# FrancisGregoryNg/Gaussian_Process_Optimization

Hardware: AMD Instinct MI355X
Metric: GP fit+predict iters/sec at N=16384 D=8 (higher is better)
Workload: dtype f64; 1 GPU; C3 (BASELINE.json configs[2]): N=16384, D=8 RBF iso, fit (K, Cholesky, alpha, LML) + predict mean/var at M=10000 candidates + EI arg-best; candidates_total=10000, candidates_this_rank=10000, entry_point=gp_fit_predict, kernel=RBF, fit=replicated on every rank (does not shard, SURVEY.md 8e), torch_imported=False, launcher=single process, emulate_fp64=0

## Files before the change

### gaussian_process_optimization_amd/csrc/api_core.hip

```cpp
#include "api_internal.h"

thread_local std::string g_err;

static thread_local bool g_note_set = false;
static thread_local std::string g_note_msg;

int fail(int code, const char *fmt, ...) {
    char buf[512];
    va_list ap;
    va_start(ap, fmt);
    vsnprintf(buf, sizeof buf, fmt, ap);
    va_end(ap);
    g_err = buf;
    if (g_note_set) {
        g_err += " [after: " + g_note_msg + "]";
        g_note_set = false;
    }
    return code;
}

void gp_note_hip(hipError_t e, const char *what, const char *file, int line) {
    if (e == hipSuccess || g_note_set) return;
    char buf[512];
    snprintf(buf, sizeof buf, "%s -> %s (%s:%d)", what, hipGetErrorString(e), file, line);
// ... 310 lines not shown
    {"panel_tiles", &gp_ctx::panel_tiles, OPT_RANGE, 1, 64},
    {"inner_tiles", &gp_ctx::inner_tiles, OPT_RANGE, 1, 2},
    {"inner_min_rows", &gp_ctx::inner_min_rows, OPT_FLOOR, 0},
    {"own_keep_per_row", &gp_ctx::own_keep_per_row, OPT_FLOOR, 0},
    {"own_keep_pipe_pct", &gp_ctx::own_keep_pipe_pct, OPT_RANGE, 0, 400},
    {"own_keep_base", &gp_ctx::own_keep_base, OPT_FLOOR, 0},
    {"lookahead", &gp_ctx::lookahead, OPT_BOOL},
    {"lookahead_min_tiles", &gp_ctx::lookahead_min_tiles, OPT_FLOOR, 0},
    {"pipe_start_pct", &gp_ctx::pipe_start_pct, OPT_RANGE, -1, 100},
    {"small_below", &gp_ctx::small_below, OPT_RAW},
    {"pipe_stages_grad", &gp_ctx::pipe_stages_grad, OPT_FLOOR, 0},
    {"pipe_start_pct_grad", &gp_ctx::pipe_start_pct_grad, OPT_RANGE, 0, 100},
    {"pipe_stages", &gp_ctx::pipe_stages, OPT_FLOOR, 0},
    {"lauum_panels", &gp_ctx::lauum_panels, OPT_RAW},
    {"side_alpha", &gp_ctx::side_alpha, OPT_RAW},
    {"pair_panels", &gp_ctx::pair_panels, OPT_BOOL},
    {"pair_tri", &gp_ctx::pair_tri, OPT_RAW},
    {"fmin_direct", &gp_ctx::fmin_direct, OPT_RAW},
    {"chain_small_below", &gp_ctx::chain_small_below, OPT_RAW},
    {"waves8", &gp_ctx::waves8, OPT_BOOL},
    {"stagger", &gp_ctx::stagger, OPT_RAW},
    {"trsm_rows64", &gp_ctx::trsm_rows64, OPT_RAW},
    {"rns_group_fit", &gp_ctx::rns_group_fit, OPT_RANGE, 1, 16},
    {"rns_group", &gp_ctx::rns_group, OPT_RANGE, 1, 16},
    {"emulate_fit", &gp_ctx::emulate_fit, OPT_BOOL},
    {"emulate_fp64", &gp_ctx::emulate_fp64, OPT_BOOL},
    {"rows_build", &gp_ctx::rows_build, OPT_RANGE, -1, 1},
    {"rows_nt", &gp_ctx::rows_nt, OPT_RANGE, -1, 1},
};

// ... 246 lines not shown
```

### gaussian_process_optimization_amd/csrc/api_factor.hip

```cpp
#include "api_internal.h"

void build_ky(gp_ctx *g, const Members &m, bool jittered) {
    launch_kbuild(g->s, m.A, m.lda, g->dX, g->N, g->Npad, m.kp[0], m.diag[0], 0, m.nb, m.sA, m.kpt, m.diag_tab);
    if (jittered) launch_add_diag(g->s, m.A, m.lda, g->N, m.jit[0], m.nb, m.sA, m.jit_tab);
    launch_set_rhs(g->s, m.A, m.lda, g->dY, g->N, g->Npad, g->P, m.nb, m.sA);
}

static int chain_step(gp_ctx *g, hipStream_t s, const Members &m, int j, int J1, int R1) {
    double *A = m.A, *invL = m.invL;
    const long lda = m.lda;
    if (g->inner_tiles >= 2 && m.nb == 1 && j + 1 < J1 && R1 - (j + 2) >= g->inner_min_rows) {
        launch_potrf_pair(s, A, lda, j, invL, m.info);
        launch_trsm2(s, A, lda, j, invL, j + 2, R1);
        if (j + 2 < J1)
            gemm(g, s, 1, A, lda, A + (long)j * GP_TILE, lda, A + (long)j * GP_TILE, lda, 1, 2 * GP_TILE,
                 TileSet{0, R1, j + 2, J1, 1});
        return j + 2;
    }
    launch_potrf_tile(s, A, lda, j, invL, m.info, m.nb, m.sA, m.sI, 4);
    gemm(g, s, 0, A, lda, A + (long)j * GP_TILE, lda, invL + (long)j * GP_TILE * GP_TILE, GP_TILE, 0, GP_TILE,
         TileSet{j + 1, R1, j, j + 1, 0}, member_opt(m, inplace_opt(), m.sA, m.sA, m.sI));
    if (j + 1 < J1)
        gemm(g, s, 1, A, lda, A + (long)j * GP_TILE, lda, A + (long)j * GP_TILE, lda, 1, GP_TILE, TileSet{0, R1, j + 1, J1, 1},
             member_opt(m, GemmOpt(), m.sA, m.sA, m.sA));
// ... 144 lines not shown
            mid_next = 0;
            if (p.edge(J + 3 + Gf) < p.nt) {
                GP_NOTE(hipStreamWaitEvent(sfar, la_event(g, EV_CONV, J), 0));
                rlaunch(sfar, Jg, J1, p.edge(J + 3 + Gf), p.nt, first);
                GP_NOTE(hipEventRecord(la_event(g, EV_FAR, gi), sfar));
                far_issued[gi] = true;
            }
        }
        if (mid_Jg >= 0 && mid_next < Gf) {
            rlaunch(sb, mid_Jg, mid_end, p.edge(mid_base + mid_next), p.edge(mid_base + mid_next + 1), mid_first);
            ++mid_next;
        }
    }
};

int factor_lookahead(gp_ctx *g, const PredPipe &pp) {
    int rc;
    if ((rc = ensure_bulk_stream(g))) return rc;
    const LaPlan p = la_plan(g, pp);
    const int nt = p.nt;
    hipStream_t sp = g->s_panel, sb = g->s_bulk;
    hipStream_t spred = pp.on ? g->s_pred : nullptr, sfar = p.Gf > 1 ? g->s_pred : nullptr;
    if ((rc = reserve_panel_inv(g, p.W, nt))) return rc;
    Members cm = ctx_members(g);
    cm.W = p.W;
    record_wait(g, EV_MISC, 0, g->s, {sp, sb, g->s_inv, spred, sfar});
    if (pp.on && pp.init) pp.init(spred);
    EmuTrail emu{g, p, cm};
    if (p.emu && (rc = emu.prepare())) return rc;
    int next_pred = 0;
    int own_prev = nt;
    for (int J = 0; J < p.nJ; ++J) {
        const int J0 = p.pb[J], J1 = p.pb[J + 1], J2 = p.pb[J + 2];
        for (int j = J0; j < J1;) j = chain_step(g, sp, cm, j, J1, p.R1);
        record_wait(g, EV_CHAIN, J, sp, {g->s_inv});
        build_panel_inv_one(g, g->s_inv, J, p.W, nt);
        if (J < p.pstages) GP_NOTE(hipEventRecord(la_event(g, EV_INVP, J), g->s_inv));
        if (pp.on && J >= p.pred_start) release_stages(g, p, pp, cm, J, &next_pred);
        if (J1 >= nt) break;
        const int oc = p.emu ? nt : first_owned_column(nt, J2, p.W, own_prev, g->own_keep_base, g->own_keep_per_row,
                                                       g->own_keep_pipe_pct, pp.on && J >= p.pred_start);
        own_prev = nt - oc;
        if (oc < nt && J >= 1) panel_update(g, sp, cm, J0, J1, TileSet{0, p.R1, oc, nt, 1});
        if (J >= 1) GP_NOTE(hipStreamWaitEvent(sp, la_event(g, EV_BULK, J - 1), 0));
        panel_update(g, sp, cm, J0, J1, TileSet{0, p.R1, J1, J2, 1});
        if (oc < nt && J == 0)
            panel_update(g, sp, cm, J0, J1, TileSet{0, p.R1, oc, nt, 1});
        if (J2 >= nt) continue;
        GP_NOTE(hipStreamWaitEvent(sb, la_event(g, EV_CHAIN, J), 0));
        if (p.emu) emu.update(J);
        else trail_fp64(g, p, cm, J, oc);
    }
    record_wait(g, EV_MISC, 1, sp, {g->s});
    record_wait(g, EV_MISC, 2, sb, {g->s});
    if (sfar) record_wait(g, EV_MISC, 7, sfar, {g->s});
    g->pipe_done = p.pstages;
    if (spred) record_wait(g, EV_MISC, 3, spred, {g->s});
    record_wait(g, EV_MISC, 4, g->s_inv, {g->s});
// ... 104 lines not shown
        pp->phase = "cholesky+potri_stages";
        pp->rest_phase = "potri_solve_rest";
        pp->flops = (double)N * N * N / 3.0;
        pp->stages = g->pipe_stages_grad;
        if (pp->stages <= 0) pp->stages = std::max(1, (nJ * 36 + 50) / 100);
        pp->start_pct = g->pipe_start_pct_grad;
    }
    return 0;
}

static int factor_attempt(gp_ctx *g, const PredPipe &pp, const double *diag_add, const double *jitter) {
    const double N = (double)g->N;
    const int nt = (int)(g->Npad / GP_TILE);
    g->lr_valid = false;
    g->jitter_try = *jitter;
    int ph = phase_begin(g, "kbuild", 0.0, 8.0 * N * g->D + 8.0 * N * N / 2);
    Members m = ctx_members(g);
    m.diag = diag_add;
    m.jit = jitter;
    build_ky(g, m, *jitter != 0.0);
    phase_end(g, ph);
    HIPCHK(hipMemsetAsync(g->dInfo, 0, sizeof(int) * 4, g->s));
    ph = phase_begin(g, pp.on ? pp.phase : "cholesky", pp.on ? pp.flops : N * N * N / 3.0, 0.0);
    const bool la = pp.on || (g->lookahead && nt > g->panel_tiles && (nt > g->lookahead_min_tiles || emu_fit_applies(g)));
    const int rc = la ? factor_lookahead(g, pp) : factor(g);
    if (rc) return rc;
    phase_end(g, ph);
    return 0;
}

static int rest_stages(gp_ctx *g, const PredPipe &pp, bool *side_alpha) {
    if (g->pipe_done >= pp.nJ) return 0;
    const int phr = phase_begin(g, pp.rest_phase, 0.0, 0.0);
    const int rci = ensure_panel_inv(g);
    if (rci) return rci;
    *side_alpha = g->s_inv && g->side_alpha;
    hipEvent_t eI = la_event(g, EV_MISC, 5);
    if (*side_alpha) GP_NOTE(hipEventRecord(eI, g->s));
    solve_rows(g, ctx_members(g), pp.mt, pp.trapezoid, g->pipe_done);
    if (*side_alpha) {
        GP_NOTE(hipStreamWaitEvent(g->s_inv, eI, 0));
        alpha_lml(g, g->s_inv, ctx_members(g));
        GP_NOTE(hipEventRecord(la_event(g, EV_MISC, 6), g->s_inv));
    }
    phase_end(g, phr);
    return 0;
}

int fit_impl(gp_ctx *g, int maxtries, Pipe kind, int include_noise) {
    HIPCHK(hipSetDevice(g->device));
    QuiesceOnError guard{g};
    const long N = g->N, Npad = g->Npad;
    const int P = g->P;
    int rc;
    PredPipe pp;
    if (kind != Pipe::None && (rc = make_pipe(g, kind, &pp))) return rc;
    double diag_add, diag0;
    ky_diag(g->kp, g->noise, &diag_add, &diag0);
    g->nphases = 0;
    g->emu_off_call = false;
    fit_dropped(g);

    double jitter = 0.0;
    int tries = 0;
    for (int info = 0, bad = 0;;) {
        if ((rc = factor_attempt(g, pp, &diag_add, &jitter))) return rc;
        if ((rc = factor_status(g, g->emulate_fp64 && !g->emu_off_call, &info, &bad))) return rc;
// ... 5 lines not shown
            continue;
        }
        if (info == 0) break;
        g->invp_valid = false;
        const int rcl = ladder_step(diag0, maxtries, info, &jitter, &tries);
        if (rcl == GP_ERR_NOT_PD_DIAG) return fail(rcl, "not pd: non-positive diagonal elements");
        if (rcl) {
            g_err = "not positive definite, even with jitter.";
            return rcl;
        }
        g->nphases = 0;
    }
    g->jitter = jitter;

    bool side_alpha = false;
    if (pp.on && (rc = rest_stages(g, pp, &side_alpha))) return rc;
    if (kind == Pipe::Identity) {
        if ((rc = wi_lauum(g))) return rc;
        g->wi_valid = true;
        g->w_in_t2 = true;
    }
    int ph = phase_begin(g, "alpha_lml", 2.0 * (double)N * N * P, 8.0 * (double)N * N / 2);
    if (side_alpha) {
        GP_NOTE(hipStreamWaitEvent(g->s, la_event(g, EV_MISC, 6), 0));
    } else {
        if ((rc = ensure_panel_inv(g))) return rc;
        alpha_lml(g, g->s, ctx_members(g));
    }
    phase_end(g, ph);
    if (kind == Pipe::Candidates) {
        ph = phase_begin(g, "reduce", 0.0, 8.0 * (double)N * g->M);
        launch_predict_reduce(g->s, g->dT2, Npad, g->M, N, g->dA + Npad * Npad, Npad, P, g->kp.variance,
                              include_noise ? g->noise : 0.0, g->dMean, g->dVar);
        phase_end(g, ph);
    }

    std::vector<double> sc(SCAL_DOT.off + P);
    HIPCHK(hipMemcpyAsync(sc.data(), g->dScal, sizeof(double) * sc.size(), hipMemcpyDeviceToHost, g->s));
    GP_SYNC(g->s);
    g->logdet = sc[SCAL_LOGDET.off];
    g->lml = lml_from_scalars(N, P, sc.data());
    g->fitted = true;
    if (kind == Pipe::Candidates) {
        g->predicted = true;
        g->predicted_noise = include_noise ? 1 : 0;
    }
    guard.armed = false;
    return 0;
// ... 41 lines not shown
```

### gaussian_process_optimization_amd/csrc/api_internal.h

```cpp
#pragma once
#include "gphip_internal.h"
#include "../../include/gphip.h"

#include <hip/hip_ext.h>
#include <rccl/rccl.h>

#include <algorithm>
#include <array>
#include <cmath>
#include <cstdarg>
#include <cstdio>
#include <cstdlib>
#include <cstring>
#include <functional>
#include <map>
#include <mutex>
#include <set>
#include <string>
#include <type_traits>
#include <vector>

extern thread_local std::string g_err;
int fail(int code, const char *fmt, ...);

// ... 108 lines not shown
    __attribute__((noinline)) int grow(long n) {
        const hipError_t e = alloc(n);
        if (e == hipSuccess) return 0;
        return std::is_same<T, double>::value ? fail(GP_ERR_HIP, "hipMalloc(%ld doubles) -> %s", n, hipGetErrorString(e))
                                              : fail(GP_ERR_HIP, "hipMalloc(%ld bytes) -> %s", n * (long)sizeof(T), hipGetErrorString(e));
    }
};

struct gp_ctx {
    int device = 0;
    hipStream_t s = nullptr;
    hipStream_t s_panel = nullptr;
    hipStream_t s_bulk = nullptr;
    int bulk_reserved = -1;
    hipStream_t s_inv = nullptr, s_pred = nullptr;
    std::vector<hipEvent_t> la_events[6];
    bool ev_error = false;
    long N = 0, Npad = 0;
    int D = 0, P = 0;
    DevBuf<double> dX, dY;
    DevBuf<double> dA;
    DevBuf<double> dInvL;
    DevBuf<double> dAlpha;
    DevBuf<double> dW;
    DevBuf<double> dMu;
    DevBuf<int> dInfo;
    DevBuf<double> dScal;
    DevBuf<double> dRedV;
    DevBuf<long long> dRedI;
    long capN = 0;
    int capP = 0;
// ... 4 lines not shown
    double jitter = 0.0, lml = 0.0, logdet = 0.0;
    double fmin = 0.0;
    bool fitted = false;
    bool fmin_valid = false;
    bool wi_valid = false;
    bool li_valid = false;
    long rows_calls_since_fit = 0;
    bool w_in_t2 = false;
    bool invp_valid = false;
    bool lr_valid = false;
    bool predicted = false;
    long M = 0;
    DevBuf<double> dXs;
    DevBuf<double> dT;
    DevBuf<double> dMean, dVar, dAcq;
    int predicted_noise = -1;
    DevBuf<double> dWi;
    DevBuf<double> dT2;
    DevBuf<double> dLi;
    DevBuf<double> dRows;
    DevBuf<unsigned int> dRowsCounter;
    double *hRowsOut = nullptr;
    double rows_ticket = 0.0;
    unsigned int rows_counter_base = 0;
    std::vector<double> lp_cache;
    int lp_cache_nb = -1;
    long rows_fused_calls = 0, rows_fallback_calls = 0;
    int rows_build = -1;
    int rows_nt = -1;
    DevBuf<double> dLp;
// ... 15 lines not shown
    Phase phases[MAX_PHASES];
    int nphases = 0;
    bool profiling = false;
    int profile_class = 0;
    std::vector<hipEvent_t> gemm_events;
    std::vector<hipEvent_t> rns_events;
    size_t rns_ev_used = 0;
    double rns_ops = 0.0;
    std::vector<long> gemm_tiles;
    std::map<std::array<int, 5>, DevBuf<short>> tile_lists;
    int supertile = 8;
    int small_below = 1400;
    int chain_small_below = 400;
    int lauum_panels = 1;
    int side_alpha = 1;
    int pair_panels = 1;
    int pair_tri = 2;
    int fmin_direct = 0;
    int trsm_rows64 = 32;
    int waves8 = 1;
    int stagger = 3;
    int pipe_stages_grad = 0, pipe_start_pct_grad = 40;
    int pipe_stages = 0;
    int pipe_done = 0;
    int pipe_start_pct = -1;
    std::vector<int> gemm_K;
    size_t gemm_ev_used = 0;
    long gemm_launches = 0;
    double gemm_flops = 0.0;
    double gemm_flops_all = 0.0;
// ... 91 lines not shown
    int nt256 = 0;
};

struct RnsSolveOpt {
    bool trapezoid = false;
    int eS = -1;
    signed char *Wr = nullptr;
    long wpitch = 0, wplane = 0;
};

struct DevStreams {
    hipStream_t s = nullptr, panel = nullptr, bulk = nullptr, inv = nullptr, pred = nullptr;
    int reserved = -1;
};

enum { EV_CHAIN = 0, EV_BULK = 1, EV_INVP = 2, EV_MISC = 3, EV_FAR = 4, EV_CONV = 5 };

void shutdown_all();
int make_bulk_stream(int device, int reserve, hipStream_t *out);
int get_streams(int device, int reserve, DevStreams *out);
int phase_begin(gp_ctx *g, const char *name, double flops, double bytes);
void phase_end(gp_ctx *g, int id);
void gemm(gp_ctx *g, hipStream_t s, int mode, double *C, long ldc, const double *A, long lda, const double *B, long ldb, int b_mul, int K, TileSet ts, const GemmOpt &o = GemmOpt());
void rns_gemm(gp_ctx *g, hipStream_t s, const signed char *A, long lda, long a_plane, const signed char *B, long ldb, long b_plane, signed char *R, int mt_all, int nt_all, int mt, int c0, int c1, int K, int first, int tri = 0);
void destroy_ctx_events(gp_ctx *g);
void build_ky(gp_ctx *g, const Members &m, bool jittered);
void factor_buf(gp_ctx *g, const Members &m, int nt, int R1, bool side_inv = false);
int factor(gp_ctx *g);
void alpha_lml(gp_ctx *g, hipStream_t s, const Members &m);
void ky_diag(const KernParams &kp, double noise, double *diag_add, double *diag0);
int ladder_step(double diag0, int maxtries, int info, double *jitter, int *tries);
int factor_status(gp_ctx *g, bool emu, int *info, int *bad);
double lml_from_scalars(long N, int P, const double *scal);
void build_panel_inv_one(gp_ctx *g, hipStream_t s, int J, int W, int nt);
int rns_prepare(gp_ctx *g, double jitter, RnsGeom *r);
void rns_convert_panel(gp_ctx *g, hipStream_t s, const RnsGeom &r, int J, int *flag);
int factor_lookahead(gp_ctx *g, const PredPipe &pp = PredPipe());
int ensure_bulk_stream(gp_ctx *g);
hipEvent_t la_event(gp_ctx *g, int kind, size_t i);
int la_events_ok(gp_ctx *g);
int reserve_panel_inv(gp_ctx *g, int W, int nt);
int ensure_panel_inv(gp_ctx *g);
void identity_blocks(hipStream_t s, double *T, long n, int nb);
void panel_inv_members(gp_ctx *g, const Members &m);
void solve_step(gp_ctx *g, hipStream_t s, const Members &m, int J, int rows);
void solve_rows(gp_ctx *g, const Members &m, int mt, int trapezoid, int J_from = 0);
int solve_rows_rns(gp_ctx *g, double *T, double *S, int mt, const RnsSolveOpt &opt = RnsSolveOpt());
int fit_impl(gp_ctx *g, int maxtries, Pipe kind, int include_noise);
int run_predict(gp_ctx *g, int include_noise, bool tiles_only = false);
int ensure_out(gp_ctx *g);
struct AcqSpec { int type; double par, fmin, y_mean, y_std; };
struct LpSpec { int transform; const double *Xb; int nb; const double *r0, *s0; };
int check_acq(const gp_ctx *g, const AcqSpec &a);
int check_lp(const LpSpec &lp);
int check_sense(int sense);
int check_k(int k);
int check_exclude(const int64_t *exclude, int nex, int64_t M);
static inline double acq_empty(int sense) { return sense > 0 ? -INFINITY : INFINITY; }
struct LpBatch { double *X = nullptr, *r = nullptr, *s = nullptr; };
static inline LpBatch lp_slots(const gp_ctx *g) { return LpBatch{g->dLp + LP_X.off, g->dLp + LP_R.off, g->dLp + LP_S.off}; }
RowsAcq rows_acq(const AcqSpec &a, const LpSpec *lp, const LpBatch &b);
// ... 19 lines not shown
```

### gaussian_process_optimization_amd/csrc/api_predict.hip

```cpp
#include "api_internal.h"

extern "C" int gp_set_candidates(gp_t *g, const double *Xs, int64_t M) {
    if (!g || !Xs) return fail(GP_ERR_ARG, "null argument");
    GP_DEAD_CHECK(g);
    if (!g->have_data) return fail(GP_ERR_STATE, "gp_set_data first");
    if (M < 1) return fail(GP_ERR_ARG, "M < 1");
    HIPCHK(hipSetDevice(g->device));
    GP_SYNC(g->s);
    int rc;
    if ((rc = g->dXs.reserve((long)M * g->D))) return rc;
    HIPCHK(hipMemcpy(g->dXs, Xs, sizeof(double) * M * g->D, hipMemcpyHostToDevice));
    g->M = M;
    g->predicted = false;
    return 0;
}

int run_predict(gp_ctx *g, int include_noise, bool tiles_only) {
    if (!g->fitted) return fail(GP_ERR_STATE, "gp_fit first");
    if (g->M < 1) return fail(GP_ERR_STATE, "gp_set_candidates first");
    HIPCHK(hipSetDevice(g->device));
    const long M = g->M, N = g->N, Npad = g->Npad;
    const int P = g->P;
    int rc;
    g->nphases = 0;
// ... 12 lines not shown
        ph = phase_begin(g, "reduce", 0.0, 8.0 * (double)N * M);
        launch_predict_reduce(g->s, g->dT2, Npad, M, N, g->dA + Npad * Npad, Npad, P, g->kp.variance,
                              include_noise ? g->noise : 0.0, g->dMean, g->dVar);
        phase_end(g, ph);
        g->predicted = true;
        g->predicted_noise = include_noise ? 1 : 0;
        return 0;
    }
    for (long m0 = 0; m0 < M; m0 += mc_max) {
        const long mc = std::min(mc_max, M - m0);
        const long mcpad = round_up(mc, GP_TILE);
        int ph = phase_begin(g, "cross_k", 0.0, 8.0 * (double)(N + mc) * g->D + 8.0 * (double)N * mc);
        launch_cross_k(g->s, g->dT, Npad, g->dXs + m0 * g->D, mc, mcpad, g->dX, g->N, Npad, g->kp);
        phase_end(g, ph);
        ph = phase_begin(g, g->emulate_fp64 ? "cand_solve_emulated" : "cand_solve", (double)N * N * mc, 0.0);
        if (g->emulate_fp64) {
            rc = solve_rows_rns(g, g->dT, g->dT2, (int)(mcpad / GP_TILE));
            if (rc == GP_ERR_RANGE) {
                ++g->emu_fallbacks;
                launch_cross_k(g->s, g->dT, Npad, g->dXs + m0 * g->D, mc, mcpad, g->dX, g->N, Npad, g->kp);
                solve_rows(g, ctx_members(g), (int)(mcpad / GP_TILE), 0);
            } else if (rc) {
                return rc;
            }
        } else {
            solve_rows(g, ctx_members(g), (int)(mcpad / GP_TILE), 0);
        }
        phase_end(g, ph);
        ph = phase_begin(g, "reduce", 0.0, 8.0 * (double)N * mc);
        launch_predict_reduce(g->s, g->dT2, Npad, mc, N, g->dA + Npad * Npad, Npad, P, g->kp.variance,
                              include_noise ? g->noise : 0.0, g->dMean + m0 * P, g->dVar + m0);
        phase_end(g, ph);
    }
    g->predicted = true;
    g->predicted_noise = include_noise ? 1 : 0;
    return 0;
}

int ensure_out(gp_ctx *g) {
    const long need = g->M * (long)std::max(1, g->P);
    if (g->dAcq.cap >= need) return 0;
    for (DevBuf<double> *b : {&g->dMean, &g->dVar, &g->dAcq}) b->release();
    int rc;
    if ((rc = g->dMean.reserve(need))) return rc;
    if ((rc = g->dVar.reserve(need))) return rc;
    return g->dAcq.reserve(need);
// ... 258 lines not shown
```

### gaussian_process_optimization_amd/csrc/api_solve.hip

```cpp
#include "api_internal.h"


static void panel_inv_steps(gp_ctx *g, hipStream_t s, double *Wb, long PB, const double *Lb, long lda, const double *Ib, int Wp,
                            GemmOpt o, long sL, long sI) {
    for (int b = 0; b < Wp; ++b) {
        o.inplace = 1;
        o.sB = sI;
        gemm(g, s, 0, Wb, PB, Wb + (long)b * GP_TILE, PB, Ib + (long)b * GP_TILE * GP_TILE, GP_TILE, 0, GP_TILE,
             TileSet{0, b + 1, b, b + 1, 0}, o);
        if (b + 1 < Wp) {
            o.inplace = 0;
            o.sB = sL;
            gemm(g, s, 1, Wb, PB, Wb + (long)b * GP_TILE, PB, Lb + (long)b * GP_TILE, lda, 1, GP_TILE,
                 TileSet{0, b + 1, b + 1, Wp, 0}, o);
        }
    }
}

int reserve_panel_inv(gp_ctx *g, int W, int nt) {
    const long PB = (long)W * GP_TILE, n = (long)((nt + W - 1) / W) * PB * PB;
    const int rc = g->dInvP.reserve(n);
    return rc ? rc : g->dInvPw.reserve(n);
}

// ... 62 lines not shown
    o.k_end_tri = 1;
    o.b_sub = J0;
    gemm(g, s, 0, m.T2, Npad, m.T + (long)J0 * GP_TILE, Npad, m.invP + (long)J * PB * PB, PB, 1, (J1 - J0) * GP_TILE,
         TileSet{0, rows, J0, J1, 0}, member_opt(m, o, m.sT, m.sT, m.sP));
}
static void rows_update(gp_ctx *g, hipStream_t s, const Members &m, int J0, int J1, int rows, int c0, int c1) {
    gemm(g, s, 1, m.T, g->Npad, m.T2 + (long)J0 * GP_TILE, g->Npad, m.A + (long)J0 * GP_TILE, m.lda, 1, (J1 - J0) * GP_TILE,
         TileSet{0, rows, c0, c1, 0}, member_opt(m, GemmOpt(), m.sT, m.sT, m.sA));
}
void solve_step(gp_ctx *g, hipStream_t s, const Members &m, int J, int rows) {
    const int nt = (int)(g->Npad / GP_TILE), J0 = J * m.W, J1 = std::min(J0 + m.W, nt);
    panel_solve(g, s, m, J, rows);
    if (J1 < nt) rows_update(g, s, m, J0, J1, rows, J1, nt);
}

void solve_rows(gp_ctx *g, const Members &m, int mt, int trapezoid, int J_from) {
    const int nt = (int)(g->Npad / GP_TILE), W = m.W;
    hipStream_t s = g->s;
    for (int J = J_from; J * W < nt;) {
        const int J0 = J * W, J1 = std::min(J0 + W, nt), J2 = std::min(J1 + W, nt);
        const int rows = trapezoid ? std::min(mt, J1) : mt;
        const bool two = g->pair_panels && !trapezoid && J2 > J1 && J2 < nt;
        if (!two) {
            solve_step(g, s, m, J, rows);
            ++J;
            continue;
        }
        panel_solve(g, s, m, J, rows);
        rows_update(g, s, m, J0, J1, rows, J1, J2);
        panel_solve(g, s, m, J + 1, rows);
        rows_update(g, s, m, J0, J2, rows, J2, nt);
        J += 2;
    }
}

void lauum(gp_ctx *g, const Members &m) {
    const long Npad = g->Npad;
    const int nt = (int)(Npad / GP_TILE);
    hipStream_t s = g->s;
    GemmOpt o;
    o.k_tri = 1;
    if (g->lauum_panels) {
        GP_NOTE(hipMemsetAsync(m.Wi, 0, sizeof(double) * (Npad * Npad + (m.nb - 1) * m.sT), s));
        const int W = g->panel_tiles;
        for (int k0 = 0; k0 < nt; k0 += W) {
// ... 94 lines not shown
```

### gaussian_process_optimization_amd/csrc/gphip_internal.h

```cpp
#pragma once
#include <hip/hip_runtime.h>
#include <stdint.h>
#include <algorithm>
#include <string>
#include <vector>

#define GP_TILE 128
#define GP_MAX_RHS 128

typedef double double4_t __attribute__((ext_vector_type(4)));
typedef double double2_t __attribute__((ext_vector_type(2)));

void gp_note_hip(hipError_t e, const char *what, const char *file, int line);
#define GP_NOTE(call) gp_note_hip((call), #call, __FILE__, __LINE__)
#define GP_LAUNCH(kernel, grid, block, lds, stream, ...)                                   \
    do {                                                                                   \
        (void)hipGetLastError();  \
        hipLaunchKernelGGL(kernel, grid, block, lds, stream, __VA_ARGS__);                 \
        gp_note_hip(hipGetLastError(), #kernel, __FILE__, __LINE__);                       \
    } while (0)

#define GP_MAX_D 64
struct KernParams {
    int kernel;
// ... 104 lines not shown
    int rows64 = 0;
    int pair = 0;
};
std::vector<short> build_tile_list(const TileSet &ts, int S);
void launch_gemm_nt(hipStream_t s, int mode, double *C, long ldc, const double *A, long lda,
                    const double *B, long ldb, int b_mul, int K, TileSet ts, const GemmOpt &o = GemmOpt());

void launch_potrf_tile(hipStream_t s, double *A, long lda, int t, double *invL, int *info, int nb = 1, long sA = 0, long sI = 0,
                       int sInfo = 0);
void launch_potrf_pair(hipStream_t s, double *A, long lda, int t, double *invL, int *info);
void launch_trsm2(hipStream_t s, double *A, long lda, int t, const double *invL, int r0, int r1);
void potrf_set_debug_lds(int bytes);


void launch_kbuild(hipStream_t s, double *A, long lda, const double *X, long N, long Npad, const KernParams &kp, double diag_add,
                   int full, int nb = 1, long sA = 0, const KernParams *kpt = nullptr, const double *diag_tab = nullptr);
void launch_set_rhs(hipStream_t s, double *A, long lda, const double *Y, long N, long Npad, int P, int nb = 1, long sA = 0);
void launch_cross_k(hipStream_t s, double *T, long ldt, const double *Xs, long M, long Mpad,
                    const double *X, long N, long Npad, const KernParams &kp);

void launch_cross_k_rows(hipStream_t s, double *T, long ldt, const double *Xs, int M, const double *X, long N, long Npad,
                         const KernParams &kp);

void launch_logdet(hipStream_t s, const double *A, long lda, long N, double *out, int nb = 1, long sA = 0, long so = 0);
void launch_rhs_sumsq(hipStream_t s, const double *A, long lda, long N, long Npad, int P, double *out);

void launch_trsv_backward(hipStream_t s, const double *L, long lda, const double *invP, int W, long Npad, const double *Z, long ldz,
                          int P, double *Aout, double *w, int nb = 1, long sL = 0, long sP = 0, long sV = 0);

void launch_predict_reduce(hipStream_t s, const double *T, long ldt, long M, long N, const double *Z,
                           long ldz, int P, double kss, double noise_add, double *mean, double *var);

void launch_train_mean(hipStream_t s, const double *X, long N, const KernParams &kp, const double *alpha,
                       double *mu);
void launch_train_mean_identity(hipStream_t s, const double *Y, const double *alpha, double d, long N, double *mu);
void launch_min(hipStream_t s, const double *v, long n, double *out);

void launch_acq(hipStream_t s, int type, double par, double fmin, double y_mean, double y_std,
                const double *mean, const double *var, long M, double *out);
void launch_argbest(hipStream_t s, const double *v, long n, int sense, double *best_val, long long *best_idx,
                    double *scratch_val, long long *scratch_idx);

void launch_small_forward_solve(hipStream_t s, const double *L, long lda, const double *invP, int W, long Npad, double *T,
                                double *S, long ldt, int M);
void launch_small_wi_product(hipStream_t s, const double *Wi, long ldw, long Npad, const double *Kx, long ldk, int M,
                             double *beta, long ldb);
// ... 73 lines not shown
```

### gaussian_process_optimization_amd/csrc/kbuild.hip

```cpp
#include "gphip_internal.h"

#define k_of_r2 gp_k_of_r2
template <int FP>
__device__ __forceinline__ double gower_factor_pair(int kernel, double variance, double dx, int disc) {
    const double r = disc ? (dx != 0.0 ? 1.0 : 0.0) : fabs(dx);
    return gp_k_of_r2_pair<FP>(kernel, variance, r * r);
}
__device__ __forceinline__ double gower_factor(int kernel, double variance, double dx, int disc) {
    return gower_factor_pair<0>(kernel, variance, dx, disc);
}

__device__ __forceinline__ void stage_rows_T(double *dst, const double *X, long row0, long N, int D,
                                             const double *ls, int tid) {
    for (int idx = tid; idx < GP_TILE * D; idx += 256) {
        const int r = idx / D, d = idx - r * D;
        const long g = row0 + r;
        dst[d * GP_TILE + r] = (g < N) ? X[g * D + d] / ls[d] : 0.0;
    }
}

template <int DU, int FP>
__device__ __forceinline__ void kbuild_body(double *A, long lda, const double *X, long N, long Npad, const KernParams &kp,
                                            double diag_add, int full, int nt) {
    extern __shared__ __attribute__((aligned(16))) double sm[];
    const int DS = DU > 0 ? DU : kp.D;
    double *xi = sm;
    double *xj = sm + (long)DS * GP_TILE;
    __shared__ double ils[GP_MAX_D];
    const int tid = threadIdx.x;
    int tm, tn;
    if (full) {
        tm = blockIdx.x / nt;
        tn = blockIdx.x % nt;
    } else {
        const long t = blockIdx.x;
        tm = (int)((sqrt(8.0 * (double)t + 1.0) - 1.0) * 0.5);
        while ((long)tm * (tm + 1) / 2 > t) --tm;
        while ((long)(tm + 1) * (tm + 2) / 2 <= t) ++tm;
        tn = (int)(t - (long)tm * (tm + 1) / 2);
    }
    if (tid < kp.D) ils[tid] = kp_div(kp, tid);
    __syncthreads();
    stage_rows_T(xi, X, (long)tm * GP_TILE, N, kp.D, ils, tid);
    stage_rows_T(xj, X, (long)tn * GP_TILE, N, kp.D, ils, tid);
    if (DU > 0)
        for (int idx = kp.D * GP_TILE + tid; idx < DU * GP_TILE; idx += 256) xi[idx] = xj[idx] = 0.0;
    __syncthreads();

    const int cx = (tid & 63) * 2;
    const int ry = tid >> 6;
    const long gc = (long)tn * GP_TILE + cx;
    double2_t bq[DU > 0 ? DU : 1];
    if (DU > 0) {
#pragma unroll
// ... 38 lines not shown
        if (gr >= N) {
            out[0] = (gr == gc) ? 1.0 : 0.0;
            out[1] = (gr == gc + 1) ? 1.0 : 0.0;
        } else {
            if (gc >= N) out[0] = 0.0;
            else if (gr == gc) out[0] = (kp.gower ? out[0] : kp.variance) + diag_add;
            if (gc + 1 >= N) out[1] = 0.0;
            else if (gr == gc + 1) out[1] = (kp.gower ? out[1] : kp.variance) + diag_add;
        }
        *(double2_t *)(A + gr * lda + gc) = out;
    }
}

template <int DU, int FP>
__global__ __launch_bounds__(256) void kbuild_kernel(double *A, long lda, const double *X, long N, long Npad,
                                                     KernParams kp, double diag_add, int full, int nt) {
    kbuild_body<DU, FP>(A, lda, X, N, Npad, kp, diag_add, full, nt);
}
template <int DU, int FP>
__global__ __launch_bounds__(256) void kbuild_batch_kernel(double *A, long lda, long sA, const double *X, long N, long Npad,
                                                           const KernParams *kpt, const double *diag_add, int nt) {
    const long z = blockIdx.z;
    kbuild_body<DU, FP>(A + z * sA, lda, X, N, Npad, kpt[z], diag_add[z], 0, nt);
}

static void launch_kbuild_members(hipStream_t s, double *A, long lda, long sA, const double *X, long N, long Npad, int DU, int fp,
                                  size_t shm, const KernParams *kpt, const double *diag_tab, int nb);
#define KB_LAUNCH_PAIR(kernel, DU, fp, ...)                       \
    do {                                                          \
        if (fp) GP_LAUNCH((kernel<DU, 1>), __VA_ARGS__);          \
        else GP_LAUNCH((kernel<DU, 0>), __VA_ARGS__);             \
    } while (0)

void launch_kbuild(hipStream_t s, double *A, long lda, const double *X, long N, long Npad, const KernParams &kp, double diag_add,
                   int full, int nb, long sA, const KernParams *kpt, const double *diag_tab) {
    const int nt = (int)(Npad / GP_TILE);
    const long nblk = full ? (long)nt * nt : (long)nt * (nt + 1) / 2;
    const int DU = kp.gower ? 0 : (kp.D <= 8 ? 8 : (kp.D <= 16 ? 16 : 0));
    const size_t shm = (size_t)2 * (DU ? DU : kp.D) * GP_TILE * sizeof(double);
    const int fp = GP_FAMILY_PAIR(kp.kernel);
    if (nb > 1) return launch_kbuild_members(s, A, lda, sA, X, N, Npad, DU, fp, shm, kpt, diag_tab, nb);
    if (DU == 8)
        KB_LAUNCH_PAIR(kbuild_kernel, 8, fp, dim3((unsigned)nblk), dim3(256), shm, s, A, lda, X, N, Npad, kp, diag_add, full, nt);
    else if (DU == 16)
        KB_LAUNCH_PAIR(kbuild_kernel, 16, fp, dim3((unsigned)nblk), dim3(256), shm, s, A, lda, X, N, Npad, kp, diag_add, full, nt);
    else
        KB_LAUNCH_PAIR(kbuild_kernel, 0, fp, dim3((unsigned)nblk), dim3(256), shm, s, A, lda, X, N, Npad, kp, diag_add, full, nt);
}

__device__ __forceinline__ void set_rhs_body(double *A, long lda, const double *Y, long N, long Npad, int P) {
    const long i = (long)blockIdx.x * blockDim.x + threadIdx.x;
    const int p = blockIdx.y;
    if (i >= Npad) return;
    A[(Npad + p) * lda + i] = (p < P && i < N) ? Y[i * P + p] : 0.0;
}
__global__ void set_rhs_kernel(double *A, long lda, const double *Y, long N, long Npad, int P) {
    set_rhs_body(A, lda, Y, N, Npad, P);
}
__global__ void set_rhs_batch_kernel(double *A, long lda, long sA, const double *Y, long N, long Npad, int P) {
    set_rhs_body(A + (long)blockIdx.z * sA, lda, Y, N, Npad, P);
}

// ... 141 lines not shown
```

### gaussian_process_optimization_amd/csrc/solve.hip

```cpp
#include "gphip_internal.h"
#include "../../include/gphip.h"
#include <algorithm>

__device__ __forceinline__ double wave_sum(double v) {
#pragma unroll
    for (int o = 32; o > 0; o >>= 1) v += __shfl_down(v, o);
    return v;
}

template <int NT>
__device__ __forceinline__ double block_sum(double v, double *sh) {
    const int lane = threadIdx.x & 63, w = threadIdx.x >> 6;
    v = wave_sum(v);
    if (lane == 0) sh[w] = v;
    __syncthreads();
    double r = 0.0;
    if (threadIdx.x == 0) {
        for (int i = 0; i < NT / 64; ++i) r += sh[i];
        sh[0] = r;
    }
    __syncthreads();
    r = sh[0];
    __syncthreads();
    return r;
// ... 183 lines not shown
            m = fma(x[0], y[0], m);
            m = fma(x[1], y[1], m);
        }
        if ((N & 1) && threadIdx.x == 0) m = fma(t[N - 1], z[N - 1], m);
        m = block_sum<256>(m, sh);
        if (threadIdx.x == 0) mean[c * P + p] = m;
    }
}
void launch_predict_reduce(hipStream_t s, const double *T, long ldt, long M, long N, const double *Z, long ldz, int P,
                           double kss, double noise_add, double *mean, double *var) {
    if (M <= 0) return;
    GP_LAUNCH(predict_reduce_kernel, dim3((unsigned)M), dim3(256), 0, s, T, ldt, N, Z, ldz, P, kss, noise_add,
                       mean, var);
}

#define k_of_r2_s gp_k_of_r2
#define TM_SPLIT 8
__global__ __launch_bounds__(256) void train_mean_kernel(const double *X, long N, KernParams kp, const double *alpha,
                                                         double *part) {
    extern __shared__ __attribute__((aligned(16))) double sm[];
    double *xi = sm;
    double *xj = sm + (long)kp.D * GP_TILE;
    double *aj = xj + (long)kp.D * GP_TILE;
    __shared__ double red[256];
    const int tid = threadIdx.x;
    const int r = tid & 127, h = tid >> 7;
    const long row0 = (long)blockIdx.x * GP_TILE;
    const long ntile = (N + GP_TILE - 1) / GP_TILE;
    for (int idx = tid; idx < GP_TILE * kp.D; idx += 256) {
        const int rr = idx / kp.D, d = idx - rr * kp.D;
// ... 133 lines not shown
```

Baseline: 14.70 fit+predict iters/s.

## Start Cholesky chain on head tiles early and overlap prediction reduce with solve

The kernel-matrix build is split into a head block of panel tiles, which is built first and signalled with an event, and the remaining tiles. The panel stream can therefore begin the first Cholesky chain while the rest of K is still being built. Separately, the predictive mean/variance reduction is split into partial chunks that run on the prediction stream as solved row ranges of the candidate triangular solve become final. A short last kernel then finishes the tail and writes the outputs. This adds events, a per-candidate accumulator buffer (M*256*(1+P) doubles) and extra kernel launches in exchange for hiding kbuild and reduce latency behind other work.

```diff
diff --git a/gaussian_process_optimization_amd/csrc/api_core.hip b/gaussian_process_optimization_amd/csrc/api_core.hip
--- a/gaussian_process_optimization_amd/csrc/api_core.hip
+++ b/gaussian_process_optimization_amd/csrc/api_core.hip
@@ -348,6 +348,8 @@
     {"pipe_stages", &gp_ctx::pipe_stages, OPT_FLOOR, 0},
     {"lauum_panels", &gp_ctx::lauum_panels, OPT_RAW},
     {"side_alpha", &gp_ctx::side_alpha, OPT_RAW},
+    {"early_chain", &gp_ctx::early_chain, OPT_BOOL},
+    {"reduce_overlap", &gp_ctx::reduce_overlap, OPT_BOOL},
     {"pair_panels", &gp_ctx::pair_panels, OPT_BOOL},
     {"pair_tri", &gp_ctx::pair_tri, OPT_RAW},
     {"fmin_direct", &gp_ctx::fmin_direct, OPT_RAW},
diff --git a/gaussian_process_optimization_amd/csrc/api_factor.hip b/gaussian_process_optimization_amd/csrc/api_factor.hip
--- a/gaussian_process_optimization_amd/csrc/api_factor.hip
+++ b/gaussian_process_optimization_amd/csrc/api_factor.hip
@@ -1,6 +1,17 @@
 #include "api_internal.h"
 
-void build_ky(gp_ctx *g, const Members &m, bool jittered) {
+void build_ky(gp_ctx *g, const Members &m, bool jittered, int head_tiles) {
+    if (head_tiles > 0 && m.nb == 1) {
+        const long N = g->N, h = std::min((long)head_tiles * GP_TILE, N);
+        launch_kbuild(g->s, m.A, m.lda, g->dX, N, g->Npad, m.kp[0], m.diag[0], 0, 1, 0, nullptr, nullptr, 0, head_tiles);
+        if (jittered) launch_add_diag(g->s, m.A, m.lda, h, m.jit[0]);
+        launch_set_rhs(g->s, m.A, m.lda, g->dY, N, g->Npad, g->P);
+        GP_NOTE(hipEventRecord(la_event(g, EV_MISC, 8), g->s));
+        launch_kbuild(g->s, m.A, m.lda, g->dX, N, g->Npad, m.kp[0], m.diag[0], 0, 1, 0, nullptr, nullptr, head_tiles,
+                      (int)(g->Npad / GP_TILE));
+        if (jittered && N > h) launch_add_diag(g->s, m.A + h * (m.lda + 1), m.lda, N - h, m.jit[0]);
+        return;
+    }
     launch_kbuild(g->s, m.A, m.lda, g->dX, g->N, g->Npad, m.kp[0], m.diag[0], 0, m.nb, m.sA, m.kpt, m.diag_tab);
     if (jittered) launch_add_diag(g->s, m.A, m.lda, g->N, m.jit[0], m.nb, m.sA, m.jit_tab);
     launch_set_rhs(g->s, m.A, m.lda, g->dY, g->N, g->Npad, g->P, m.nb, m.sA);
@@ -182,7 +193,7 @@
     }
 };
 
-int factor_lookahead(gp_ctx *g, const PredPipe &pp) {
+int factor_lookahead(gp_ctx *g, const PredPipe &pp, bool early) {
     int rc;
     if ((rc = ensure_bulk_stream(g))) return rc;
     const LaPlan p = la_plan(g, pp);
@@ -192,7 +203,8 @@
     if ((rc = reserve_panel_inv(g, p.W, nt))) return rc;
     Members cm = ctx_members(g);
     cm.W = p.W;
-    record_wait(g, EV_MISC, 0, g->s, {sp, sb, g->s_inv, spred, sfar});
+    if (early) GP_NOTE(hipStreamWaitEvent(sp, la_event(g, EV_MISC, 8), 0));
+    record_wait(g, EV_MISC, 0, g->s, {early ? nullptr : sp, sb, g->s_inv, spred, sfar});
     if (pp.on && pp.init) pp.init(spred);
     EmuTrail emu{g, p, cm};
     if (p.emu && (rc = emu.prepare())) return rc;
@@ -210,6 +222,7 @@
                                                        g->own_keep_pipe_pct, pp.on && J >= p.pred_start);
         own_prev = nt - oc;
         if (oc < nt && J >= 1) panel_update(g, sp, cm, J0, J1, TileSet{0, p.R1, oc, nt, 1});
+        if (early && J == 0) GP_NOTE(hipStreamWaitEvent(sp, la_event(g, EV_MISC, 0), 0));
         if (J >= 1) GP_NOTE(hipStreamWaitEvent(sp, la_event(g, EV_BULK, J - 1), 0));
         panel_update(g, sp, cm, J0, J1, TileSet{0, p.R1, J1, J2, 1});
         if (oc < nt && J == 0)
@@ -344,22 +357,24 @@
     const int nt = (int)(g->Npad / GP_TILE);
     g->lr_valid = false;
     g->jitter_try = *jitter;
+    const bool la = pp.on || (g->lookahead && nt > g->panel_tiles && (nt > g->lookahead_min_tiles || emu_fit_applies(g)));
+    const bool early = g->early_chain && la && nt > g->panel_tiles && !emu_fit_applies(g);
+    if (early) HIPCHK(hipMemsetAsync(g->dInfo, 0, sizeof(int) * 4, g->s));
     int ph = phase_begin(g, "kbuild", 0.0, 8.0 * N * g->D + 8.0 * N * N / 2);
     Members m = ctx_members(g);
     m.diag = diag_add;
     m.jit = jitter;
-    build_ky(g, m, *jitter != 0.0);
+    build_ky(g, m, *jitter != 0.0, early ? g->panel_tiles : 0);
     phase_end(g, ph);
-    HIPCHK(hipMemsetAsync(g->dInfo, 0, sizeof(int) * 4, g->s));
+    if (!early) HIPCHK(hipMemsetAsync(g->dInfo, 0, sizeof(int) * 4, g->s));
     ph = phase_begin(g, pp.on ? pp.phase : "cholesky", pp.on ? pp.flops : N * N * N / 3.0, 0.0);
-    const bool la = pp.on || (g->lookahead && nt > g->panel_tiles && (nt > g->lookahead_min_tiles || emu_fit_applies(g)));
-    const int rc = la ? factor_lookahead(g, pp) : factor(g);
+    const int rc = la ? factor_lookahead(g, pp, early) : factor(g);
     if (rc) return rc;
     phase_end(g, ph);
     return 0;
 }
 
-static int rest_stages(gp_ctx *g, const PredPipe &pp, bool *side_alpha) {
+static int rest_stages(gp_ctx *g, const PredPipe &pp, bool *side_alpha, ReduceOverlap *ro) {
     if (g->pipe_done >= pp.nJ) return 0;
     const int phr = phase_begin(g, pp.rest_phase, 0.0, 0.0);
     const int rci = ensure_panel_inv(g);
@@ -367,7 +382,7 @@
     *side_alpha = g->s_inv && g->side_alpha;
     hipEvent_t eI = la_event(g, EV_MISC, 5);
     if (*side_alpha) GP_NOTE(hipEventRecord(eI, g->s));
-    solve_rows(g, ctx_members(g), pp.mt, pp.trapezoid, g->pipe_done);
+    solve_rows(g, ctx_members(g), pp.mt, pp.trapezoid, g->pipe_done, ro);
     if (*side_alpha) {
         GP_NOTE(hipStreamWaitEvent(g->s_inv, eI, 0));
         alpha_lml(g, g->s_inv, ctx_members(g));
@@ -380,7 +395,7 @@
 int fit_impl(gp_ctx *g, int maxtries, Pipe kind, int include_noise) {
     HIPCHK(hipSetDevice(g->device));
     QuiesceOnError guard{g};
-    const long N = g->N, Npad = g->Npad;
+    const long N = g->N;
     const int P = g->P;
     int rc;
     PredPipe pp;
@@ -416,7 +431,9 @@
     g->jitter = jitter;
 
     bool side_alpha = false;
-    if (pp.on && (rc = rest_stages(g, pp, &side_alpha))) return rc;
+    ReduceOverlap ro;
+    if (kind == Pipe::Candidates && (rc = reduce_begin(g, g->M, &ro))) return rc;
+    if (pp.on && (rc = rest_stages(g, pp, &side_alpha, &ro))) return rc;
     if (kind == Pipe::Identity) {
         if ((rc = wi_lauum(g))) return rc;
         g->wi_valid = true;
@@ -432,8 +449,7 @@
     phase_end(g, ph);
     if (kind == Pipe::Candidates) {
         ph = phase_begin(g, "reduce", 0.0, 8.0 * (double)N * g->M);
-        launch_predict_reduce(g->s, g->dT2, Npad, g->M, N, g->dA + Npad * Npad, Npad, P, g->kp.variance,
-                              include_noise ? g->noise : 0.0, g->dMean, g->dVar);
+        reduce_finish(g, ro, g->M, include_noise, g->dMean, g->dVar);
         phase_end(g, ph);
     }
 
diff --git a/gaussian_process_optimization_amd/csrc/api_internal.h b/gaussian_process_optimization_amd/csrc/api_internal.h
--- a/gaussian_process_optimization_amd/csrc/api_internal.h
+++ b/gaussian_process_optimization_amd/csrc/api_internal.h
@@ -146,7 +146,7 @@
     hipStream_t s_bulk = nullptr;
     int bulk_reserved = -1;
     hipStream_t s_inv = nullptr, s_pred = nullptr;
-    std::vector<hipEvent_t> la_events[6];
+    std::vector<hipEvent_t> la_events[7];
     bool ev_error = false;
     long N = 0, Npad = 0;
     int D = 0, P = 0;
@@ -181,6 +181,7 @@
     DevBuf<double> dXs;
     DevBuf<double> dT;
     DevBuf<double> dMean, dVar, dAcq;
+    DevBuf<double> dRedAcc;
     int predicted_noise = -1;
     DevBuf<double> dWi;
     DevBuf<double> dT2;
@@ -226,6 +227,8 @@
     int chain_small_below = 400;
     int lauum_panels = 1;
     int side_alpha = 1;
+    int early_chain = 1;
+    int reduce_overlap = 1;
     int pair_panels = 1;
     int pair_tri = 2;
     int fmin_direct = 0;
@@ -347,7 +350,15 @@
     int reserved = -1;
 };
 
-enum { EV_CHAIN = 0, EV_BULK = 1, EV_INVP = 2, EV_MISC = 3, EV_FAR = 4, EV_CONV = 5 };
+enum { EV_CHAIN = 0, EV_BULK = 1, EV_INVP = 2, EV_MISC = 3, EV_FAR = 4, EV_CONV = 5, EV_RED = 6 };
+
+struct ReduceOverlap {
+    long M = 0;
+    const double *Z = nullptr;
+    long ldz = 0;
+    long done = 0;
+    int chunks = 0;
+};
 
 void shutdown_all();
 int make_bulk_stream(int device, int reserve, hipStream_t *out);
@@ -357,7 +368,7 @@
 void gemm(gp_ctx *g, hipStream_t s, int mode, double *C, long ldc, const double *A, long lda, const double *B, long ldb, int b_mul, int K, TileSet ts, const GemmOpt &o = GemmOpt());
 void rns_gemm(gp_ctx *g, hipStream_t s, const signed char *A, long lda, long a_plane, const signed char *B, long ldb, long b_plane, signed char *R, int mt_all, int nt_all, int mt, int c0, int c1, int K, int first, int tri = 0);
 void destroy_ctx_events(gp_ctx *g);
-void build_ky(gp_ctx *g, const Members &m, bool jittered);
+void build_ky(gp_ctx *g, const Members &m, bool jittered, int head_tiles = 0);
 void factor_buf(gp_ctx *g, const Members &m, int nt, int R1, bool side_inv = false);
 int factor(gp_ctx *g);
 void alpha_lml(gp_ctx *g, hipStream_t s, const Members &m);
@@ -368,7 +379,7 @@
 void build_panel_inv_one(gp_ctx *g, hipStream_t s, int J, int W, int nt);
 int rns_prepare(gp_ctx *g, double jitter, RnsGeom *r);
 void rns_convert_panel(gp_ctx *g, hipStream_t s, const RnsGeom &r, int J, int *flag);
-int factor_lookahead(gp_ctx *g, const PredPipe &pp = PredPipe());
+int factor_lookahead(gp_ctx *g, const PredPipe &pp = PredPipe(), bool early = false);
 int ensure_bulk_stream(gp_ctx *g);
 hipEvent_t la_event(gp_ctx *g, int kind, size_t i);
 int la_events_ok(gp_ctx *g);
@@ -377,7 +388,9 @@
 void identity_blocks(hipStream_t s, double *T, long n, int nb);
 void panel_inv_members(gp_ctx *g, const Members &m);
 void solve_step(gp_ctx *g, hipStream_t s, const Members &m, int J, int rows);
-void solve_rows(gp_ctx *g, const Members &m, int mt, int trapezoid, int J_from = 0);
+void solve_rows(gp_ctx *g, const Members &m, int mt, int trapezoid, int J_from = 0, ReduceOverlap *ro = nullptr);
+int reduce_begin(gp_ctx *g, long M, ReduceOverlap *ro);
+void reduce_finish(gp_ctx *g, const ReduceOverlap &ro, long M, int include_noise, double *mean, double *var);
 int solve_rows_rns(gp_ctx *g, double *T, double *S, int mt, const RnsSolveOpt &opt = RnsSolveOpt());
 int fit_impl(gp_ctx *g, int maxtries, Pipe kind, int include_noise);
 int run_predict(gp_ctx *g, int include_noise, bool tiles_only = false);
diff --git a/gaussian_process_optimization_amd/csrc/api_predict.hip b/gaussian_process_optimization_amd/csrc/api_predict.hip
--- a/gaussian_process_optimization_amd/csrc/api_predict.hip
+++ b/gaussian_process_optimization_amd/csrc/api_predict.hip
@@ -50,6 +50,7 @@
         launch_cross_k(g->s, g->dT, Npad, g->dXs + m0 * g->D, mc, mcpad, g->dX, g->N, Npad, g->kp);
         phase_end(g, ph);
         ph = phase_begin(g, g->emulate_fp64 ? "cand_solve_emulated" : "cand_solve", (double)N * N * mc, 0.0);
+        ReduceOverlap ro;
         if (g->emulate_fp64) {
             rc = solve_rows_rns(g, g->dT, g->dT2, (int)(mcpad / GP_TILE));
             if (rc == GP_ERR_RANGE) {
@@ -60,12 +61,12 @@
                 return rc;
             }
         } else {
-            solve_rows(g, ctx_members(g), (int)(mcpad / GP_TILE), 0);
+            if ((rc = reduce_begin(g, mc, &ro))) return rc;
+            solve_rows(g, ctx_members(g), (int)(mcpad / GP_TILE), 0, 0, &ro);
         }
         phase_end(g, ph);
         ph = phase_begin(g, "reduce", 0.0, 8.0 * (double)N * mc);
-        launch_predict_reduce(g->s, g->dT2, Npad, mc, N, g->dA + Npad * Npad, Npad, P, g->kp.variance,
-                              include_noise ? g->noise : 0.0, g->dMean + m0 * P, g->dVar + m0);
+        reduce_finish(g, ro, mc, include_noise, g->dMean + m0 * P, g->dVar + m0);
         phase_end(g, ph);
     }
     g->predicted = true;
diff --git a/gaussian_process_optimization_amd/csrc/api_solve.hip b/gaussian_process_optimization_amd/csrc/api_solve.hip
--- a/gaussian_process_optimization_amd/csrc/api_solve.hip
+++ b/gaussian_process_optimization_amd/csrc/api_solve.hip
@@ -100,7 +100,40 @@
     if (J1 < nt) rows_update(g, s, m, J0, J1, rows, J1, nt);
 }
 
-void solve_rows(gp_ctx *g, const Members &m, int mt, int trapezoid, int J_from) {
+int reduce_begin(gp_ctx *g, long M, ReduceOverlap *ro) {
+    *ro = ReduceOverlap();
+    if (!g->reduce_overlap || !g->s_pred || M < 1) return 0;
+    const int rc = g->dRedAcc.reserve(M * 256 * (1 + (long)g->P));
+    if (rc) return rc;
+    ro->M = M;
+    ro->Z = g->dA + g->Npad * g->Npad;
+    ro->ldz = g->Npad;
+    return 0;
+}
+static void reduce_chunk(gp_ctx *g, ReduceOverlap *ro, int Jend) {
+    if (!ro || ro->M < 1) return;
+    const long c1 = std::min((long)Jend * GP_TILE, g->N & ~1L) / 512 * 512;
+    if (c1 <= ro->done) return;
+    GP_NOTE(hipEventRecord(la_event(g, EV_RED, 2 * ro->chunks), g->s));
+    GP_NOTE(hipStreamWaitEvent(g->s_pred, la_event(g, EV_RED, 2 * ro->chunks), 0));
+    launch_predict_reduce_part(g->s_pred, g->dT2, g->Npad, ro->M, g->N, ro->done, c1, ro->Z, ro->ldz, g->P, g->dRedAcc);
+    GP_NOTE(hipEventRecord(la_event(g, EV_RED, 2 * ro->chunks + 1), g->s_pred));
+    ro->done = c1;
+    ++ro->chunks;
+}
+void reduce_finish(gp_ctx *g, const ReduceOverlap &ro, long M, int include_noise, double *mean, double *var) {
+    const long Npad = g->Npad;
+    const double noise_add = include_noise ? g->noise : 0.0;
+    if (ro.chunks == 0) {
+        launch_predict_reduce(g->s, g->dT2, Npad, M, g->N, g->dA + Npad * Npad, Npad, g->P, g->kp.variance, noise_add, mean, var);
+        return;
+    }
+    GP_NOTE(hipStreamWaitEvent(g->s, la_event(g, EV_RED, 2 * (ro.chunks - 1) + 1), 0));
+    launch_predict_reduce_last(g->s, g->dT2, Npad, ro.M, g->N, ro.done, ro.Z, ro.ldz, g->P, g->dRedAcc, g->kp.variance, noise_add, mean,
+                               var);
+}
+
+void solve_rows(gp_ctx *g, const Members &m, int mt, int trapezoid, int J_from, ReduceOverlap *ro) {
     const int nt = (int)(g->Npad / GP_TILE), W = m.W;
     hipStream_t s = g->s;
     for (int J = J_from; J * W < nt;) {
@@ -108,13 +141,18 @@
         const int rows = trapezoid ? std::min(mt, J1) : mt;
         const bool two = g->pair_panels && !trapezoid && J2 > J1 && J2 < nt;
         if (!two) {
-            solve_step(g, s, m, J, rows);
+            panel_solve(g, s, m, J, rows);
+            if (J1 < nt) {
+                reduce_chunk(g, ro, J1);
+                rows_update(g, s, m, J0, J1, rows, J1, nt);
+            }
             ++J;
             continue;
         }
         panel_solve(g, s, m, J, rows);
         rows_update(g, s, m, J0, J1, rows, J1, J2);
         panel_solve(g, s, m, J + 1, rows);
+        reduce_chunk(g, ro, J2);
         rows_update(g, s, m, J0, J2, rows, J2, nt);
         J += 2;
     }
diff --git a/gaussian_process_optimization_amd/csrc/gphip_internal.h b/gaussian_process_optimization_amd/csrc/gphip_internal.h
--- a/gaussian_process_optimization_amd/csrc/gphip_internal.h
+++ b/gaussian_process_optimization_amd/csrc/gphip_internal.h
@@ -142,7 +142,8 @@
 
 
 void launch_kbuild(hipStream_t s, double *A, long lda, const double *X, long N, long Npad, const KernParams &kp, double diag_add,
-                   int full, int nb = 1, long sA = 0, const KernParams *kpt = nullptr, const double *diag_tab = nullptr);
+                   int full, int nb = 1, long sA = 0, const KernParams *kpt = nullptr, const double *diag_tab = nullptr, int tc0 = 0,
+                   int tc1 = -1);
 void launch_set_rhs(hipStream_t s, double *A, long lda, const double *Y, long N, long Npad, int P, int nb = 1, long sA = 0);
 void launch_cross_k(hipStream_t s, double *T, long ldt, const double *Xs, long M, long Mpad,
                     const double *X, long N, long Npad, const KernParams &kp);
@@ -158,6 +159,11 @@
 
 void launch_predict_reduce(hipStream_t s, const double *T, long ldt, long M, long N, const double *Z,
                            long ldz, int P, double kss, double noise_add, double *mean, double *var);
+#define REDUCE_PART_ROWS 8
+void launch_predict_reduce_part(hipStream_t s, const double *T, long ldt, long M, long N, long c0, long c1, const double *Z, long ldz,
+                                int P, double *acc);
+void launch_predict_reduce_last(hipStream_t s, const double *T, long ldt, long M, long N, long c0, const double *Z, long ldz, int P,
+                                const double *acc, double kss, double noise_add, double *mean, double *var);
 
 void launch_train_mean(hipStream_t s, const double *X, long N, const KernParams &kp, const double *alpha,
                        double *mu);
diff --git a/gaussian_process_optimization_amd/csrc/kbuild.hip b/gaussian_process_optimization_amd/csrc/kbuild.hip
--- a/gaussian_process_optimization_amd/csrc/kbuild.hip
+++ b/gaussian_process_optimization_amd/csrc/kbuild.hip
@@ -21,7 +21,7 @@
 
 template <int DU, int FP>
 __device__ __forceinline__ void kbuild_body(double *A, long lda, const double *X, long N, long Npad, const KernParams &kp,
-                                            double diag_add, int full, int nt) {
+                                            double diag_add, int full, int nt, int tc0, int tc1) {
     extern __shared__ __attribute__((aligned(16))) double sm[];
     const int DS = DU > 0 ? DU : kp.D;
     double *xi = sm;
@@ -34,10 +34,18 @@
         tn = blockIdx.x % nt;
     } else {
         const long t = blockIdx.x;
-        tm = (int)((sqrt(8.0 * (double)t + 1.0) - 1.0) * 0.5);
-        while ((long)tm * (tm + 1) / 2 > t) --tm;
-        while ((long)(tm + 1) * (tm + 2) / 2 <= t) ++tm;
-        tn = (int)(t - (long)tm * (tm + 1) / 2);
+        const int w = tc1 - tc0;
+        const long tri = (long)w * (w + 1) / 2;
+        if (t < tri) {
+            tm = (int)((sqrt(8.0 * (double)t + 1.0) - 1.0) * 0.5);
+            while ((long)tm * (tm + 1) / 2 > t) --tm;
+            while ((long)(tm + 1) * (tm + 2) / 2 <= t) ++tm;
+            tn = (int)(t - (long)tm * (tm + 1) / 2) + tc0;
+            tm += tc0;
+        } else {
+            tm = tc1 + (int)((t - tri) / w);
+            tn = tc0 + (int)((t - tri) % w);
+        }
     }
     if (tid < kp.D) ils[tid] = kp_div(kp, tid);
     __syncthreads();
@@ -106,14 +114,14 @@
 
 template <int DU, int FP>
 __global__ __launch_bounds__(256) void kbuild_kernel(double *A, long lda, const double *X, long N, long Npad,
-                                                     KernParams kp, double diag_add, int full, int nt) {
-    kbuild_body<DU, FP>(A, lda, X, N, Npad, kp, diag_add, full, nt);
+                                                     KernParams kp, double diag_add, int full, int nt, int tc0, int tc1) {
+    kbuild_body<DU, FP>(A, lda, X, N, Npad, kp, diag_add, full, nt, tc0, tc1);
 }
 template <int DU, int FP>
 __global__ __launch_bounds__(256) void kbuild_batch_kernel(double *A, long lda, long sA, const double *X, long N, long Npad,
                                                            const KernParams *kpt, const double *diag_add, int nt) {
     const long z = blockIdx.z;
-    kbuild_body<DU, FP>(A + z * sA, lda, X, N, Npad, kpt[z], diag_add[z], 0, nt);
+    kbuild_body<DU, FP>(A + z * sA, lda, X, N, Npad, kpt[z], diag_add[z], 0, nt, 0, nt);
 }
 
 static void launch_kbuild_members(hipStream_t s, double *A, long lda, long sA, const double *X, long N, long Npad, int DU, int fp,
@@ -125,19 +133,24 @@
     } while (0)
 
 void launch_kbuild(hipStream_t s, double *A, long lda, const double *X, long N, long Npad, const KernParams &kp, double diag_add,
-                   int full, int nb, long sA, const KernParams *kpt, const double *diag_tab) {
+                   int full, int nb, long sA, const KernParams *kpt, const double *diag_tab, int tc0, int tc1) {
     const int nt = (int)(Npad / GP_TILE);
-    const long nblk = full ? (long)nt * nt : (long)nt * (nt + 1) / 2;
+    if (tc1 < 0 || full || nb > 1) tc0 = 0, tc1 = nt;
+    tc0 = std::max(0, std::min(tc0, nt));
+    tc1 = std::max(tc0, std::min(tc1, nt));
+    const long wr = tc1 - tc0;
+    const long nblk = full ? (long)nt * nt : wr * (wr + 1) / 2 + (long)(nt - tc1) * wr;
+    if (nblk == 0) return;
     const int DU = kp.gower ? 0 : (kp.D <= 8 ? 8 : (kp.D <= 16 ? 16 : 0));
     const size_t shm = (size_t)2 * (DU ? DU : kp.D) * GP_TILE * sizeof(double);
     const int fp = GP_FAMILY_PAIR(kp.kernel);
     if (nb > 1) return launch_kbuild_members(s, A, lda, sA, X, N, Npad, DU, fp, shm, kpt, diag_tab, nb);
     if (DU == 8)
-        KB_LAUNCH_PAIR(kbuild_kernel, 8, fp, dim3((unsigned)nblk), dim3(256), shm, s, A, lda, X, N, Npad, kp, diag_add, full, nt);
+        KB_LAUNCH_PAIR(kbuild_kernel, 8, fp, dim3((unsigned)nblk), dim3(256), shm, s, A, lda, X, N, Npad, kp, diag_add, full, nt, tc0, tc1);
     else if (DU == 16)
-        KB_LAUNCH_PAIR(kbuild_kernel, 16, fp, dim3((unsigned)nblk), dim3(256), shm, s, A, lda, X, N, Npad, kp, diag_add, full, nt);
+        KB_LAUNCH_PAIR(kbuild_kernel, 16, fp, dim3((unsigned)nblk), dim3(256), shm, s, A, lda, X, N, Npad, kp, diag_add, full, nt, tc0, tc1);
     else
-        KB_LAUNCH_PAIR(kbuild_kernel, 0, fp, dim3((unsigned)nblk), dim3(256), shm, s, A, lda, X, N, Npad, kp, diag_add, full, nt);
+        KB_LAUNCH_PAIR(kbuild_kernel, 0, fp, dim3((unsigned)nblk), dim3(256), shm, s, A, lda, X, N, Npad, kp, diag_add, full, nt, tc0, tc1);
 }
 
 __device__ __forceinline__ void set_rhs_body(double *A, long lda, const double *Y, long N, long Npad, int P) {
diff --git a/gaussian_process_optimization_amd/csrc/solve.hip b/gaussian_process_optimization_amd/csrc/solve.hip
--- a/gaussian_process_optimization_amd/csrc/solve.hip
+++ b/gaussian_process_optimization_amd/csrc/solve.hip
@@ -221,6 +221,74 @@
                        mean, var);
 }
 
+template <bool LAST>
+__global__ __launch_bounds__(256) void predict_reduce_part_kernel(const double *T, long ldt, long M, long N, long c0, long c1,
+                                                                  int rows, const double *Z, long ldz, int P, double *acc,
+                                                                  double kss, double noise_add, double *mean, double *var) {
+    __shared__ double sh[4];
+    const long i0 = (c0 >> 1) + threadIdx.x, i1 = LAST ? (N >> 1) : (c1 >> 1);
+    for (long c = (long)blockIdx.x * rows, ce = c + rows < M ? c + rows : M; c < ce; ++c) {
+        const double *t = T + c * ldt;
+        double *a = acc + c * (1 + P) * 256 + threadIdx.x;
+        double s = 0.0, m0 = 0.0;
+        if (c0 > 0) {
+            s = a[0];
+            m0 = a[256];
+        }
+        for (long i = i0; i < i1; i += 256) {
+            const double2_t x = *(const double2_t *)(t + 2 * i);
+            const double2_t y = *(const double2_t *)(Z + 2 * i);
+            s = fma(x[0], x[0], s);
+            s = fma(x[1], x[1], s);
+            m0 = fma(x[0], y[0], m0);
+            m0 = fma(x[1], y[1], m0);
+        }
+        if (LAST) {
+            if ((N & 1) && threadIdx.x == 0) {
+                s = fma(t[N - 1], t[N - 1], s);
+                m0 = fma(t[N - 1], Z[N - 1], m0);
+            }
+            s = block_sum<256>(s, sh);
+            if (threadIdx.x == 0) var[c] = (kss - s) + noise_add;
+            m0 = block_sum<256>(m0, sh);
+            if (threadIdx.x == 0) mean[c * P] = m0;
+        } else {
+            a[0] = s;
+            a[256] = m0;
+        }
+        for (int p = 1; p < P; ++p) {
+            const double *z = Z + p * ldz;
+            double m = c0 > 0 ? a[(1 + p) * 256] : 0.0;
+            for (long i = i0; i < i1; i += 256) {
+                const double2_t x = *(const double2_t *)(t + 2 * i);
+                const double2_t y = *(const double2_t *)(z + 2 * i);
+                m = fma(x[0], y[0], m);
+                m = fma(x[1], y[1], m);
+            }
+            if (LAST) {
+                if ((N & 1) && threadIdx.x == 0) m = fma(t[N - 1], z[N - 1], m);
+                m = block_sum<256>(m, sh);
+                if (threadIdx.x == 0) mean[c * P + p] = m;
+            } else {
+                a[(1 + p) * 256] = m;
+            }
+        }
+    }
+}
+void launch_predict_reduce_part(hipStream_t s, const double *T, long ldt, long M, long N, long c0, long c1, const double *Z, long ldz,
+                                int P, double *acc) {
+    if (M <= 0 || c1 <= c0 || (c0 & 511) || (c1 & 511) || c1 > (N & ~1L)) return;
+    const int rows = REDUCE_PART_ROWS;
+    GP_LAUNCH((predict_reduce_part_kernel<false>), dim3((unsigned)((M + rows - 1) / rows)), dim3(256), 0, s, T, ldt, M, N, c0, c1, rows,
+              Z, ldz, P, acc, 0.0, 0.0, (double *)nullptr, (double *)nullptr);
+}
+void launch_predict_reduce_last(hipStream_t s, const double *T, long ldt, long M, long N, long c0, const double *Z, long ldz, int P,
+                                const double *acc, double kss, double noise_add, double *mean, double *var) {
+    if (M <= 0) return;
+    GP_LAUNCH((predict_reduce_part_kernel<true>), dim3((unsigned)M), dim3(256), 0, s, T, ldt, M, N, c0, N, 1, Z, ldz, P,
+              const_cast<double *>(acc), kss, noise_add, mean, var);
+}
+
 #define k_of_r2_s gp_k_of_r2
 #define TM_SPLIT 8
 __global__ __launch_bounds__(256) void train_mean_kernel(const double *X, long N, KernParams kp, const double *alpha,
```

Result: slower. 14.46 fit+predict iters/s (-1.7%).
